# jhultman/vision3d

Measured on AMD Instinct MI355X. Metric: frames/sec SECOND fwd, 16k-pt KITTI cloud, higher is better.
Workload: dtype f16x3-scaled (fp32-class): fp32 operands split into f16 hi + lo pieces of x * s under per-tensor power-of-two scales, 3 MFMA terms (lo*hi + hi*lo + hi*hi), fp32 accumulate; relative product error 2^-22 -- the result differs from the reference's fp32 modules by fp32 summation noise: strict elementwis

## Files before the change

vision3d_amd/csrc/spconv.hip:

```cpp
#include "v3d_internal.h"

#include "sp_device.h"
#include "rb_device.h"

#define SP_RIDER_PROLOGUE(lds)                                                                        \
  if (rider.blocks && (int)blockIdx.x < rider.blocks) {                                               \
    if (threadIdx.x < V3D_BLOCK) rb_rider_run(rider, (int)blockIdx.x, (unsigned char*)(lds));         \
    return;                                                                                           \
  }                                                                                                   \
  const int bid = (int)blockIdx.x - rider.blocks;                                                     \
  [[maybe_unused]] const int nblk = (int)gridDim.x - rider.blocks;



__global__ __launch_bounds__(V3D_BLOCK) void spconv_fwd_scalar(const float* __restrict__ in,
                                                               const float* __restrict__ W,
                                                               const int* __restrict__ nbr,
                                                               const int* __restrict__ n_ptr, int cap, int K, int Cin,
                                                               int Cout, const float* __restrict__ scale,
                                                               const float* __restrict__ shift, int relu,
                                                               float* __restrict__ out) {
  const int n = min(*n_ptr, cap);
  const long long total = (long long)n * Cout;
  for (long long t = (long long)blockIdx.x * V3D_BLOCK + threadIdx.x; t < total; t += (long long)gridDim.x * V3D_BLOCK) {
// ... 931 lines not shown

template <int CIN, int COUT, int OG, int NBUF, int NMV, int ALOOK, int STAGE, int TILES, int PREC, int INS>
__device__ __forceinline__ void spconv_ring_body(const float* __restrict__ in, const unsigned short* __restrict__ wimg,
                                                 const int* __restrict__ nbr, const int n, int cap, const float* __restrict__ scale,
                                                 const float* __restrict__ shift, int relu, float* __restrict__ out, const int wg_in,
                                                 const SpScales& ss, float& vmax, unsigned short* __restrict__ out_s, const float s_next,
                                                 unsigned char* __restrict__ wb0 ) {
  constexpr int K = 27, ROUNDS = (K + OG - 1) / OG, NCW = TILES * OG;
  constexpr int LOOK = NBUF - 1;
  constexpr int ABUF = ALOOK + 1;
  constexpr int KI = CIN / 32, NB = COUT / 16;
  constexpr int NF = KI * NB * 2;
  constexpr int WBYTES = NF * 1024;
  constexpr int RB = OG * WBYTES;
  constexpr int FPM = OG * NF / NMV;
  constexpr int NSTG = (ROUNDS + 3) / 4;
  static_assert(CIN % 32 == 0 && CIN <= 128 && (OG * NF) % NMV == 0 && (LOOK - 1) * FPM < 64, "shape not covered by the ring kernel");
  static_assert(RB >= TILES * OG * NB * 4 * 64 * 4, "partials must fit one round buffer");
  static_assert(ALOOK >= 1 && ALOOK <= 4 && (ALOOK * KI * 2 <= 8 || ALOOK * KI * 2 == 12 || ALOOK * KI * 2 == 16), "gather look-ahead");
  __shared__ __attribute__((aligned(16))) unsigned char wb1[RB];
  __shared__ __attribute__((aligned(16))) unsigned char wb2[NBUF >= 3 ? RB : 16];
  __shared__ __attribute__((aligned(16))) unsigned char wb3[NBUF == 4 ? RB : 16];
  __shared__ int nbr_all[TILES * K * 16];
  __shared__ __attribute__((aligned(16))) unsigned char aslot[STAGE ? NCW * ALOOK * CIN * 64 : 16];
#define SPR_RING(i) ((i) % NBUF == 0 ? wb0 : ((i) % NBUF == 1 ? wb1 : ((i) % NBUF == 2 ? wb2 : wb3)))
  const int tid = threadIdx.x, lane = tid & 63;
  const int wv = __builtin_amdgcn_readfirstlane(tid >> 6);
  int wg = wg_in;
  {
    const int nwg = (n + 16 * TILES - 1) / (16 * TILES);
    const int qd = nwg / 8, rmd = nwg % 8, xcd = wg % 8, idx = wg / 8;
    wg = (xcd < rmd ? xcd * (qd + 1) : rmd * (qd + 1) + (xcd - rmd) * qd) + idx;
  }

  [[maybe_unused]] const int wave = wv == NCW ? 3 : (wv < 3 ? wv : 99);
  SPR_STAMP(0);
  if (wv >= NCW) {
    typedef const __attribute__((address_space(1))) void* gptr_t;
    typedef __attribute__((address_space(3))) void* lptr_t;
    const int mv = wv - NCW;
    const unsigned char* wsrc = reinterpret_cast<const unsigned char*>(wimg) + (size_t)mv * FPM * 1024 + (size_t)lane * 16;
#define SPR_DMA(R)                                                                                                  \
  {                                                                                                                 \
    const unsigned char* gsrc = wsrc + (size_t)(R) * RB;                                                            \
    _Pragma("unroll") for (int i = 0; i < FPM; i++) {                                                               \
      const bool ok = (R) * OG + (mv * FPM + i) / NF < K;                                                           \
      __builtin_amdgcn_global_load_lds((gptr_t)(gsrc + i * 1024 - (ok ? 0 : WBYTES)),                               \
                                       (lptr_t)(SPR_RING(R) + (mv * FPM + i) * 1024), 16, 0, 0);                    \
    }                                                                                                               \
  }
#pragma unroll
    for (int R = 0; R < LOOK; R++) SPR_DMA(R)
    SPR_STAMP(1);
#pragma unroll
    for (int R = 0; R < ROUNDS; R++) {
      const int younger = (ROUNDS - 1 - R) < (LOOK - 1) ? (ROUNDS - 1 - R) : (LOOK - 1);
      if (younger == 2) asm volatile("s_waitcnt vmcnt(%0)\n\ts_barrier" ::"n"(2 * FPM < 64 ? 2 * FPM : 63) : "memory");
      else if (younger == 1) asm volatile("s_waitcnt vmcnt(%0)\n\ts_barrier" ::"n"(FPM) : "memory");
      else asm volatile("s_waitcnt vmcnt(0)\n\ts_barrier" ::: "memory");
      if (R + LOOK < ROUNDS) SPR_DMA(R + LOOK)
      SPR_STAMP(3 + (R < 9 ? R : 8));
    }
#undef SPR_DMA
    __syncthreads();
    return;
  }

  const int t = wv / OG, g = wv % OG;
  int* nbr_s = nbr_all + t * K * 16;
  const int row0 = (wg * TILES + t) * 16;
  const int r = lane & 15, kg = lane >> 4;
  f32x4 araw[STAGE ? 1 : ABUF][KI * 2];
  f32x4 acc[NB];
#pragma unroll
  for (int j = 0; j < NB; j++) acc[j] = f32x4{0.f, 0.f, 0.f, 0.f};
  const int rsel = STAGE ? (lane >> 2) : r;
  const float* prow = spr_zero_row;
  auto row_ptr = [&](int src_i) {
    const int src = src_i;
    prow = (src >= 0 ? in + (size_t)src * CIN : spr_zero_row) + (STAGE ? ((lane & 3) ^ ((lane >> 5) & 1)) * 4 : (INS ? kg * 4 : kg * 8));
  };
  const unsigned slot0 = STAGE ? __builtin_amdgcn_readfirstlane(lds_addr_of(aslot) + wv * (ALOOK * CIN * 64)) : 0u;
  auto issue_chunk = [&](int ki, int Rr) {
    if constexpr (STAGE) {
      asm_dma16(prow + (ki * 2) * 16, slot0 + (Rr % ALOOK) * (CIN * 64) + (ki * 2) * 1024);
      asm_dma16(prow + (ki * 2 + 1) * 16, slot0 + (Rr % ALOOK) * (CIN * 64) + (ki * 2 + 1) * 1024);
    } else {
      f32x4 (&a)[KI * 2] = araw[Rr % ABUF];
      if constexpr (INS) {
        if (ki == 0) {
          asm_gld16(a[0], prow);
          if constexpr (CIN == 64) asm_gld16_128(a[1], prow);
          else asm_gld16_64(a[1], prow);
        } else if constexpr (KI == 2) {
          asm_gld16_64(a[2], prow);
          asm_gld16_192(a[3], prow);
        }
      } else if (ki == 0) {
        asm_gld16(a[0], prow);
        asm_gld16_16(a[1], prow);
      } else if constexpr (KI == 2) {
        asm_gld16_128(a[2], prow);
        asm_gld16_144(a[3], prow);
      }
    }
  };
  int nsrc = -1;
  {
    const bool live = row0 + r < n;
    int first[ALOOK], stage[NSTG];
#pragma unroll
    for (int i = 0; i < ALOOK; i++) first[i] = (row0 + rsel < n && i * OG + g < K) ? nbr[(size_t)(i * OG + g) * cap + row0 + rsel] : -1;
#pragma unroll
    for (int i = 0; i < NSTG; i++) {
      const int kk = (kg + 4 * i) * OG + g;
      stage[i] = (live && kk < K) ? nbr[(size_t)kk * cap + row0 + r] : -1;
    }
#pragma unroll
    for (int i = 0; i < ALOOK; i++) {
      row_ptr(first[i]);
#pragma unroll
      for (int ki = 0; ki < KI; ki++) issue_chunk(ki, i);
    }
#pragma unroll
    for (int i = 0; i < NSTG; i++)
      if ((kg + 4 * i) * OG + g < K) nbr_s[((kg + 4 * i) * OG + g) * 16 + r] = stage[i];
    if (ALOOK < ROUNDS && ALOOK * OG + g < K) nsrc = nbr_s[(ALOOK * OG + g) * 16 + rsel];
  }
  SPR_STAMP(1);
#pragma unroll
  for (int R = 0; R < ROUNDS; R++) {
    asm volatile("s_waitcnt lgkmcnt(0)\n\ts_barrier" ::: "memory");
    if (R + ALOOK < ROUNDS) row_ptr(nsrc);
    if (R + ALOOK + 1 < ROUNDS) nsrc = ((R + ALOOK + 1) * OG + g < K) ? nbr_s[((R + ALOOK + 1) * OG + g) * 16 + rsel] : -1;
    {
      const int younger = (ROUNDS - 1 - R < ALOOK - 1 ? ROUNDS - 1 - R : ALOOK - 1) * KI * 2;
      if constexpr (STAGE) {
        if (younger == 0) vm_wait<0>();
        else if (younger == 2) vm_wait<2>();
        else if (younger == 4) vm_wait<4>();
        else if (younger == 6) vm_wait<6>();
        else if (younger == 8) vm_wait<8>();
        else vm_wait<12>();
        const int sw = (r >> 3) & 1;
        const unsigned char* sl = aslot + (wv * ALOOK + R % ALOOK) * (CIN * 64) + (INS ? r * 64 + ((kg ^ sw) * 16) : (kg >> 1) * 1024 + r * 64);
#pragma unroll
        for (int ki = 0; ki < KI; ki++)
#pragma unroll
          for (int v = 0; v < 2; v++)
            araw[0][ki * 2 + v] = INS ? *reinterpret_cast<const f32x4*>(sl + (v * KI + ki) * 1024)
                                      : *reinterpret_cast<const f32x4*>(sl + ki * 2048 + ((((kg & 1) * 2 + v) ^ sw) * 16));
      } else {
        f32x4 (&ar)[KI * 2] = araw[R % ABUF];
        if (younger == 0) vm_wait_tie<0>(ar);
        else if (younger == 2) vm_wait_tie<2>(ar);
        else if (younger == 4) vm_wait_tie<4>(ar);
        else if (younger == 6) vm_wait_tie<6>(ar);
        else if (younger == 8) vm_wait_tie<8>(ar);
        else if (younger == 12) vm_wait_tie<12>(ar);
        else vm_wait_tie<16>(ar);
      }
    }
    const u32x4_t* bw = reinterpret_cast<const u32x4_t*>(SPR_RING(R) + g * WBYTES) + lane;
    u32x4_t ah[KI], al[KI], bh[KI][NB], bl[KI][NB];
#pragma unroll
    for (int ki = 0; ki < KI; ki++)
#pragma unroll
      for (int j = 0; j < NB; j++) {
        bh[ki][j] = bw[(size_t)((ki * NB + j) * 2) * 64];
        bl[ki][j] = bw[(size_t)((ki * NB + j) * 2 + 1) * 64];
      }
#pragma unroll
    for (int ki = 0; ki < KI; ki++) {
      const f32x4 v0 = araw[STAGE ? 0 : R % ABUF][ki * 2], v1 = araw[STAGE ? 0 : R % ABUF][ki * 2 + 1];
      const float x[8] = {v0.x, v0.y, v0.z, v0.w, v1.x, v1.y, v1.z, v1.w};
      split_in<PREC, INS>(x, ss.s_in, ah[ki], al[ki]);
    }
#pragma unroll
    for (int ki = 0; ki < KI; ki++) {
#pragma unroll
      for (int j = 0; j < NB; j++) acc[j] = sp_mfma<PREC>(al[ki], bh[ki][j], acc[j]);
#pragma unroll
      for (int j = 0; j < NB; j++) acc[j] = sp_mfma<PREC>(ah[ki], bl[ki][j], acc[j]);
#pragma unroll
      for (int j = 0; j < NB; j++) acc[j] = sp_mfma<PREC>(ah[ki], bh[ki][j], acc[j]);
      if (R + ALOOK < ROUNDS) {
        __builtin_amdgcn_sched_barrier(0);
        issue_chunk(ki, R + ALOOK);
        __builtin_amdgcn_sched_barrier(0);
      }
    }
#if SPR_TIMELINE
    __builtin_amdgcn_sched_barrier(0);
    SPR_STAMP(3 + (R < 9 ? R : 8));
#endif
  }
  float* part = reinterpret_cast<float*>((ROUNDS - 1) % NBUF != 0 ? wb0 : wb1) + t * (OG * NB * 4 * 64);
#pragma unroll
  for (int j = 0; j < NB; j++)
#pragma unroll
    for (int rr = 0; rr < 4; rr++) part[((g * NB + j) * 4 + rr) * 64 + lane] = acc[j][rr];
  SPR_STAMP(12);
  __syncthreads();
  SPR_STAMP(13);
  for (int it = g; it < NB * 4; it += OG) {
    const int j = it >> 2, rr = it & 3;
    const int col = j * 16 + r, row = row0 + kg * 4 + rr;
    float v = part[((0 * NB + j) * 4 + rr) * 64 + lane];
#pragma unroll
    for (int w = 1; w < OG; w++) v += part[((w * NB + j) * 4 + rr) * 64 + lane];
    if (row < n) {
      if (scale) v = v * (scale[col] * ss.undo) + shift[col];
      else if constexpr (PREC == 1) v = v * ss.undo;
      if (relu) v = fmaxf(v, 0.f);
      if constexpr (PREC == 1) vmax = fmaxf(vmax, fabsf(v));
      if (out) out[(size_t)row * COUT + col] = v;
      if (out_s) sp_store_split<PREC, COUT>(out_s, row, col, r, v, s_next);
    }
  }
  SPR_STAMP(14);
#undef SPR_RING
}

template <int CIN, int COUT, int OG, int NBUF, int NMV, int ALOOK, int STAGE, int TILES, int PREC, int INS>
__global__ __launch_bounds__((TILES * OG + NMV) * 64) void spconv_fwd_rows_ring(const float* __restrict__ in,
                                                                          const unsigned short* __restrict__ wimg,
                                                                          const int* __restrict__ nbr,
                                                                          const int* __restrict__ n_ptr, int cap,
                                                                          const float* __restrict__ scale,
                                                                          const float* __restrict__ shift, int relu,
                                                                          float* __restrict__ out, const V3dActScale as,
                                                                          unsigned short* __restrict__ out_s, const RbScanJob rider) {
  constexpr int RB0 = OG * (CIN / 32) * (COUT / 16) * 2 * 1024;
  static_assert(RB0 >= RB_SCAN_LDS, "a rider's scratch fits round buffer 0");
  __shared__ __attribute__((aligned(16))) unsigned char wb0[RB0];
  constexpr bool HOST = !(CIN == 64 && COUT == 64);
  int bid = (int)blockIdx.x, nblk = (int)gridDim.x;
  if constexpr (HOST) {
    if (rider.blocks && bid < rider.blocks) {
      if (threadIdx.x < V3D_BLOCK) rb_rider_run(rider, bid, wb0);
      return;
    }
    bid -= rider.blocks;
    nblk -= rider.blocks;
  }
  const int n = min(*n_ptr, cap);
  const int nwg = (n + 16 * TILES - 1) / (16 * TILES);
  const SpScales ss = sp_scales<PREC>(as, wimg, (size_t)27 * (CIN / 32) * (COUT / 16) * 2 * 512);
  const float s_next = (PREC == 1 && out_s) ? as.next[0] : 1.f;
  float vmax = 0.f;
  for (int g = bid; g < nwg; g += nblk) {
    spconv_ring_body<CIN, COUT, OG, NBUF, NMV, ALOOK, STAGE, TILES, PREC, INS>(in, wimg, nbr, n, cap, scale, shift, relu, out, g, ss, vmax,
                                                                              out_s, s_next, wb0);
    __syncthreads();
  }
  if constexpr (PREC == 1) sp_range_check(as, vmax, ss.limit);
}

struct SpLaunch {
  int prec;
  V3dActScale as;
  const void* in_split;
  unsigned short* out_split;
  const RbScanJob* rider;
  bool* rider_taken;
};

static RbScanJob sp_ring_rider(const SpLaunch& sl, int max_blocks) {
  if (!sl.rider || max_blocks < 1 || sl.rider->blocks > max_blocks) return RbScanJob{};
  return *sl.rider;
}

template <int CIN, int COUT, int OG, int NBUF, int NMV, int ALOOK, int STAGE, int TILES, int PREC, int INS>
static int launch_rows_ring_p(const float* in, const void* wimg, const int* nbr, const int* n_ptr, int cap,
                              const float* scale, const float* shift, int relu, float* out, hipStream_t st, const SpLaunch& sl) {
  static V3dPerDeviceInt cache;
  int* slots = cache.slot();
  if (!*slots) {
    int dev = 0, n_cu = 0, per_cu = 0;
    V3D_CHECK_HIP(hipGetDevice(&dev));
    V3D_CHECK_HIP(hipDeviceGetAttribute(&n_cu, hipDeviceAttributeMultiprocessorCount, dev));
    V3D_CHECK_HIP(hipOccupancyMaxActiveBlocksPerMultiprocessor(&per_cu, spconv_fwd_rows_ring<CIN, COUT, OG, NBUF, NMV, ALOOK, STAGE, TILES, PREC, INS>,
                                                               (TILES * OG + NMV) * 64, 0));
    *slots = std::max(8, per_cu * n_cu / 8 * 8);
  }
  const RbScanJob r = sp_ring_rider(sl, CIN == 64 && COUT == 64 ? 0 : 512);
  const int grid = std::min(v3d_ceil_div(cap, 16 * TILES), std::max(*slots - r.blocks, 8));
  hipLaunchKernelGGL((spconv_fwd_rows_ring<CIN, COUT, OG, NBUF, NMV, ALOOK, STAGE, TILES, PREC, INS>), dim3(grid + r.blocks),
                     dim3((TILES * OG + NMV) * 64), 0, st, INS ? (const float*)sl.in_split : in, (const unsigned short*)wimg, nbr, n_ptr, cap,
                     scale, shift, relu, out, sl.as, sl.out_split, r);
  if (sl.rider_taken) *sl.rider_taken = r.blocks > 0;
  V3D_CHECK_LAUNCH();
  return V3D_OK;
}
template <int CIN, int COUT, int OG, int NBUF, int NMV, int ALOOK = 2, int STAGE = 0, int TILES = 2>
static int launch_rows_ring(const float* in, const void* wimg, const int* nbr, const int* n_ptr, int cap,
                            const float* scale, const float* shift, int relu, float* out, hipStream_t st, const SpLaunch& sl) {
#define V3D_RING(P, I) launch_rows_ring_p<CIN, COUT, OG, NBUF, NMV, ALOOK, STAGE, TILES, P, I>(in, wimg, nbr, n_ptr, cap, scale, shift, relu, out, st, sl)
  if (sl.prec == V3D_PREC_F16S) return sl.in_split ? V3D_RING(1, 1) : V3D_RING(1, 0);
  return sl.in_split ? V3D_RING(0, 1) : V3D_RING(0, 0);
#undef V3D_RING
}

template <int CIN, int COUT, int PREC, int INS>
static void launch_rows_big(const float* in, const void* wimg, const int* nbr, const int* n_ptr, int cap, int K,
                            const float* scale, const float* shift, int relu, float* out, hipStream_t st, const SpLaunch& sl) {
  constexpr int NF = ((CIN + 31) / 32) * (COUT / 16) * 2;
  const size_t lds = std::max((size_t)2 * NF * 64 * 16 + (size_t)K * 64 * 4, (size_t)4 * SP_STAGE_BYTES(COUT));
  hipLaunchKernelGGL((spconv_fwd_rows_big<CIN, COUT, PREC, INS>), dim3(v3d_ceil_div(cap, 64)), dim3(V3D_BLOCK), lds, st,
                     INS ? (const float*)sl.in_split : in, (const unsigned short*)wimg, nbr, n_ptr, cap, K, scale, shift, relu, out, sl.as,
                     sl.out_split);
}

template <int CIN, int COUT, int T, int STAGE, int PREC, int INS>
static void launch_rows_kouter(const float* in, const void* wimg, const int* nbr, const int* n_ptr, int cap,
                               const float* scale, const float* shift, int relu, float* out, hipStream_t st, const SpLaunch& sl) {
  const int passes = v3d_ceil_div(cap, 16 * (T == 3 ? 2 : T) * 8);
  const int grid = passes >= 256 ? 256 : ((passes + 7) / 8) * 8;
  hipLaunchKernelGGL((spconv_fwd_rows_kouter<CIN, COUT, T, 27, STAGE, PREC, INS>), dim3(grid), dim3(512), 0, st,
                     INS ? (const float*)sl.in_split : in, (const unsigned short*)wimg, nbr, n_ptr, cap, scale, shift, relu, out, sl.as,
                     sl.out_split);
}

#define V3D_BIG_ROWS 32768
#define V3D_RING_ROWS 16384
template <int CIN, int COUT, int PREC, int INS>
static int launch_rows(const float* in, const void* wimg, const int* nbr, const int* n_ptr, int cap, int K,
                       const float* scale, const float* shift, int relu, float* out, int rows_hint, hipStream_t st,
                       const V3dDensifyOut* densify, int tiles_min, const SpLaunch& sl) {
  const int force = densify ? 1 : (rows_hint < 0 ? -rows_hint : 0);
  if constexpr (CIN >= 32 && CIN <= 64 && COUT >= 32 && COUT <= 64) {
    if (K == 27 && (force == 6 || force == 7 || force == 8 || (force == 0 && CIN == 64 && COUT == 64 && rows_hint >= V3D_BIG_ROWS))) {
      if (force == 7) launch_rows_kouter<CIN, COUT, 2, 0, PREC, INS>(in, wimg, nbr, n_ptr, cap, scale, shift, relu, out, st, sl);
      else if (force == 8) launch_rows_kouter<CIN, COUT, 2, 1, PREC, INS>(in, wimg, nbr, n_ptr, cap, scale, shift, relu, out, st, sl);
      else launch_rows_kouter<CIN, COUT, 3, 1, PREC, INS>(in, wimg, nbr, n_ptr, cap, scale, shift, relu, out, st, sl);
      V3D_CHECK_LAUNCH();
      return V3D_OK;
    }
    if (force == 5 || (force == 0 && rows_hint >= V3D_BIG_ROWS)) {
      launch_rows_big<CIN, COUT, PREC, INS>(in, wimg, nbr, n_ptr, cap, K, scale, shift, relu, out, st, sl);
      V3D_CHECK_LAUNCH();
      return V3D_OK;
    }
    if (K == 27 && (force == 10 || force == 16 || (force >= 12 && force <= 14) || (force == 0 && rows_hint <= V3D_RING_ROWS))) {
      if constexpr (CIN == 64 && COUT == 64) {
        if (force != 16) {
          const long long want = force ? 0 : (long long)rows_hint + rows_hint / 10;
          int tiles = force == 12 ? 2 : force == 13 ? 3 : force == 14 ? 4 : (want <= 32 * 256 ? 2 : want <= 48 * 256 ? 3 : 4);
          if (!force && tiles < tiles_min) tiles = tiles_min > 4 ? 4 : tiles_min;
          if (tiles == 2) return launch_rows_ring<CIN, COUT, 3, 2, 4, 1, 1, 2>(in, wimg, nbr, n_ptr, cap, scale, shift, relu, out, st, sl);
          if (tiles == 3) return launch_rows_ring<CIN, COUT, 3, 2, 4, 1, 1, 3>(in, wimg, nbr, n_ptr, cap, scale, shift, relu, out, st, sl);
          return launch_rows_ring<CIN, COUT, 3, 2, 4, 1, 1, 4>(in, wimg, nbr, n_ptr, cap, scale, shift, relu, out, st, sl);
        }
      }
      if (force != 16 && CIN == 32 && COUT == 32) return launch_rows_ring<CIN, COUT, 3, 2, 2, 2, 1>(in, wimg, nbr, n_ptr, cap, scale, shift, relu, out, st, sl);
      return launch_rows_ring<CIN, COUT, 3, 3, 2>(in, wimg, nbr, n_ptr, cap, scale, shift, relu, out, st, sl);
    }
  }
  const size_t lds = std::max((size_t)4 * (COUT / 16) * 4 * 64 * 4 + (size_t)K * 16 * 4 + 2 * SP_STAGE_BYTES(COUT),
                              (size_t)RB_SCAN_LDS);
  const RbScanJob r = sl.rider ? *sl.rider : RbScanJob{};
  hipLaunchKernelGGL((spconv_fwd_rows<CIN, COUT, PREC, INS>), dim3(v3d_ceil_div(cap, 16) + r.blocks), dim3(V3D_BLOCK), lds, st,
                     INS ? (const float*)sl.in_split : in, (const unsigned short*)wimg, nbr, n_ptr, cap, K, scale, shift, relu, out,
                     densify ? *densify : V3dDensifyOut{}, sl.as, sl.out_split, r);
  if (sl.rider_taken) *sl.rider_taken = r.blocks > 0;
  V3D_CHECK_LAUNCH();
  return V3D_OK;
}

extern "C" int v3d_sparse_conv_fwd_packed(const float* in, const void* weight_image, const int32_t* nbr,
                                           const int32_t* n_out, int cap_out, int K, int Cin, int Cout, const float* scale,
                                           const float* shift, int relu, float* out, int rows_hint, int prec,
                                           const float* act_in, const float* act_next, int32_t* range_flag,
                                           const void* in_split, void* out_split, v3d_stream_t stream) {
  const V3dActScale as{act_in, act_next, range_flag, nullptr};
  return v3d_i_sparse_conv_fwd_packed(in ? in : (const float*)in_split, weight_image, nbr, n_out, cap_out, K, Cin, Cout, scale, shift,
                                      relu, out, rows_hint, (hipStream_t)stream, nullptr, 2, prec, &as, in_split, out_split);
}

template <int PREC>
__global__ __launch_bounds__(256) void rows_split_kernel(const float* __restrict__ rows, const int* __restrict__ n_ptr, int cap, int C,
                                                         const float* __restrict__ entry, unsigned short* __restrict__ out) {
  const long long total = (long long)(n_ptr ? min(*n_ptr, cap) : cap) * C;
  const float s = PREC == 1 ? entry[0] : 1.f;
  for (long long t = (long long)blockIdx.x * 256 + threadIdx.x; t < total; t += (long long)gridDim.x * 256) {
    const long long row = t / C;
    const int c = (int)(t - row * C);
    unsigned short h, l;
    split_one<PREC>(rows[t], s, h, l);
    out[row * 2 * C + c] = h;
    out[row * 2 * C + C + c] = l;
  }
}

extern "C" int v3d_sparse_rows_split(const float* rows, const int32_t* n_rows, int cap, int C, int prec, const float* act_entry,
                                     void* out_split, v3d_stream_t stream) {
  if (!rows || !out_split || cap < 1 || C < 8 || C % 8) return V3D_EINVAL;
  if (prec == V3D_PREC_F16S ? !act_entry : prec != V3D_PREC_BF16X3) return V3D_EINVAL;
  const int blocks = (int)std::min<long long>(((long long)cap * C + 255) / 256, 4096);
  if (prec == V3D_PREC_F16S)
    hipLaunchKernelGGL(rows_split_kernel<1>, dim3(blocks), dim3(256), 0, (hipStream_t)stream, rows, n_rows, cap, C, act_entry, (unsigned short*)out_split);
  else
    hipLaunchKernelGGL(rows_split_kernel<0>, dim3(blocks), dim3(256), 0, (hipStream_t)stream, rows, n_rows, cap, C, nullptr, (unsigned short*)out_split);
  V3D_CHECK_LAUNCH();
  return V3D_OK;
}

bool v3d_i_sparse_conv_packed_supported(int Cin, int Cout) {
  static const int shapes[][2] = {{4, 16}, {16, 16}, {16, 32}, {32, 32}, {32, 64}, {64, 64}, {4, 32}, {32, 16}, {64, 32}, {64, 128}, {128, 128}};
  for (const auto& s : shapes)
    if (s[0] == Cin && s[1] == Cout) return true;
  return false;
}

int v3d_i_sparse_conv_fwd_packed(const float* in, const void* weight_image, const int32_t* nbr, const int32_t* n_out,
                                 int cap_out, int K, int Cin, int Cout, const float* scale, const float* shift, int relu,
                                 float* out, int rows_hint, hipStream_t st, const V3dDensifyOut* densify, int ring_tiles_min,
                                 int prec, const V3dActScale* act, const void* in_split, void* out_split, const RbScanJob* rider,
                                 bool* rider_taken) {
  if (rider_taken) *rider_taken = false;
  if (!in || !weight_image || !nbr || !n_out || (!out && !out_split) || cap_out < 1 || K < 1) return V3D_EINVAL;
  if ((scale == nullptr) != (shift == nullptr)) return V3D_EINVAL;
  if (!out && densify) return V3D_EINVAL;
  if (prec != V3D_PREC_BF16X3 && prec != V3D_PREC_F16S) return V3D_EINVAL;
  if (prec == V3D_PREC_F16S && (!act || !act->in || ((densify || out_split) && !act->next))) return V3D_EINVAL;
  if (in_split && Cin % 8) return V3D_EINVAL;
  SpLaunch sl;
  sl.prec = prec;
  sl.as = (prec == V3D_PREC_F16S) ? *act : V3dActScale{nullptr, nullptr, nullptr, nullptr};
  sl.in_split = in_split;
  sl.out_split = (unsigned short*)out_split;
  sl.rider = rider;
  sl.rider_taken = rider_taken;
#define V3D_GO(ci, co, P, I) \
  return launch_rows<ci, co, P, I>(in, weight_image, nbr, n_out, cap_out, K, scale, shift, relu, out, rows_hint, st, densify, ring_tiles_min, sl)
#define V3D_TRY(ci, co)                                    \
  if (Cin == ci && Cout == co) {                           \
    if constexpr ((ci) % 8 == 0) {                         \
      if (prec == V3D_PREC_F16S && in_split) V3D_GO(ci, co, 1, 1); \
      if (prec == V3D_PREC_BF16X3 && in_split) V3D_GO(ci, co, 0, 1); \
    }                                                      \
    if (prec == V3D_PREC_F16S) V3D_GO(ci, co, 1, 0);       \
    V3D_GO(ci, co, 0, 0);                                  \
  }
  V3D_TRY(4, 16)
  V3D_TRY(16, 16)
  V3D_TRY(16, 32)
  V3D_TRY(32, 32)
  V3D_TRY(32, 64)
  V3D_TRY(64, 64)
  V3D_TRY(4, 32)
  V3D_TRY(32, 16)
  V3D_TRY(64, 32)
  V3D_TRY(64, 128)
  V3D_TRY(128, 128)
#undef V3D_TRY
#undef V3D_GO
  return V3D_EUNSUPPORTED;
}

extern "C" int v3d_sparse_conv_fwd(const float* in, const float* weight, const int32_t* nbr, const int32_t* n_out,
                                   int cap_out, int K, int Cin, int Cout, const float* scale, const float* shift,
                                   int relu, float* out, int algo, v3d_stream_t stream) {
  return v3d_i_sparse_conv_fwd_exact(in, weight, nbr, n_out, cap_out, K, Cin, Cout, scale, shift, relu, out, algo, (hipStream_t)stream,
                                     nullptr, nullptr, nullptr, nullptr, nullptr);
}

int v3d_i_sparse_conv_fwd_exact(const float* in, const float* weight, const int32_t* nbr, const int32_t* n_out, int cap_out, int K,
                                int Cin, int Cout, const float* scale, const float* shift, int relu, float* out, int algo,
                                hipStream_t st, const float* next_entry, int32_t* range_flag, unsigned* seen, const RbScanJob* rider,
                                bool* rider_taken) {
  if (rider_taken) *rider_taken = false;
  if (!in || !weight || !nbr || !n_out || !out || cap_out < 1 || K < 1 || Cin < 1 || Cout < 1) return V3D_EINVAL;
  if ((scale == nullptr) != (shift == nullptr)) return V3D_EINVAL;
  if (algo != 0 && algo != 1 && algo != 3) return V3D_EINVAL;
  if (algo == 0 || algo == 3) {
    int rc = V3D_EUNSUPPORTED;
#define V3D_TRY(ci, co) \
  if (Cin == ci && Cout == co) rc = launch_wave<ci, co>(in, weight, nbr, n_out, cap_out, K, scale, shift, relu, out, st, next_entry, range_flag, seen, rider, rider_taken);
    V3D_TRY(4, 16)
    V3D_TRY(16, 16)
    V3D_TRY(16, 32)
    V3D_TRY(32, 32)
    V3D_TRY(32, 64)
    V3D_TRY(64, 64)
    V3D_TRY(4, 32)
    V3D_TRY(32, 16)
    V3D_TRY(64, 32)
    V3D_TRY(64, 128)
    V3D_TRY(128, 128)
#undef V3D_TRY
    if (rc != V3D_EUNSUPPORTED || algo == 3) return rc;
  }
  const long long total = (long long)cap_out * Cout;
  const int blocks = (int)((total + V3D_BLOCK - 1) / V3D_BLOCK);
  hipLaunchKernelGGL(spconv_fwd_scalar, dim3(blocks > 8192 ? 8192 : blocks), dim3(V3D_BLOCK), 0, st, in, weight, nbr,
                       n_out, cap_out, K, Cin, Cout, scale, shift, relu, out);
  V3D_CHECK_LAUNCH();
  return V3D_OK;
}

#define BW_MAX_SPLITS 64
#define BW_Q 128

__host__ __device__ static inline int bw_rows_per_block(int n) {
  const int r = ((n + BW_MAX_SPLITS - 1) / BW_MAX_SPLITS + 255) & ~255;
  return r < 256 ? 256 : r;
}

template <int TI, int TJ>
__global__ __launch_bounds__(V3D_BLOCK) void spconv_bwd_weight_tiles(const float* __restrict__ X,
                                                                     const float* __restrict__ dY,
                                                                     const int* __restrict__ nbr,
                                                                     const int* __restrict__ n_ptr, int cap, int Cin,
                                                                     int Cout, int groups_j,
                                                                     float* __restrict__ partial ) {
  __shared__ int q_src[4][BW_Q];
  __shared__ int q_out[4][BW_Q];
  __shared__ float red[TI * TJ * 256];
  const int n = min(*n_ptr, cap);
  const int rows_per_block = bw_rows_per_block(n);
  const int slab = blockIdx.x, k = blockIdx.y, K = gridDim.y;
  const int lo = slab * rows_per_block;
  if (lo >= n) return;
  const int hi = min(n, lo + rows_per_block);
  const int ci_base = (blockIdx.z / groups_j) * TI * 16, co_base = (blockIdx.z % groups_j) * TJ * 16;
  const int lane = threadIdx.x & 63, wave = threadIdx.x >> 6;
  const int r = lane & 15, p = lane >> 4;
  const int rows_per_wave = rows_per_block >> 2;
  const int wlo = lo + wave * rows_per_wave, whi = min(hi, wlo + rows_per_wave);
  const int* __restrict__ nk = nbr + (size_t)k * cap;
  int* qs = q_src[wave];
  int* qo = q_out[wave];

  f32x4 acc[TI][TJ];
#pragma unroll
  for (int t = 0; t < TI; t++)
#pragma unroll
    for (int u = 0; u < TJ; u++) acc[t][u] = f32x4{0.f, 0.f, 0.f, 0.f};

  auto consume = [&](int base, int valid) {
    float a[4][TI], b[4][TJ];
#pragma unroll
    for (int s4 = 0; s4 < 4; s4++) {
      const int e = 4 * s4 + p;
      const bool ok = e < valid;
      const int src = ok ? qs[base + e] : 0, o = ok ? qo[base + e] : 0;
#pragma unroll
      for (int t = 0; t < TI; t++) {
        const int ci = ci_base + 16 * t + r;
        a[s4][t] = (ok && ci < Cin) ? X[(size_t)src * Cin + ci] : 0.f;
      }
#pragma unroll
      for (int u = 0; u < TJ; u++) {
        const int co = co_base + 16 * u + r;
        b[s4][u] = (ok && co < Cout) ? dY[(size_t)o * Cout + co] : 0.f;
      }
    }
#pragma unroll
    for (int s4 = 0; s4 < 4; s4++)
#pragma unroll
      for (int t = 0; t < TI; t++)
#pragma unroll
        for (int u = 0; u < TJ; u++) acc[t][u] = __builtin_amdgcn_mfma_f32_16x16x4f32(a[s4][t], b[s4][u], acc[t][u], 0, 0, 0);
  };

  int cnt = 0;
  int src_next = (wlo < whi && wlo + lane < whi) ? nk[wlo + lane] : -1;
  for (int o0 = wlo; o0 < whi; o0 += 64) {
    const int src = src_next;
    const int o = o0 + lane;
    src_next = (o + 64 < whi) ? nk[o + 64] : -1;
    const unsigned long long live = __ballot(src >= 0);
    if (src >= 0) {
      const int pos = cnt + __popcll(live & ((1ull << lane) - 1ull));
      qs[pos] = src;
      qo[pos] = o;
    }
    cnt += __popcll(live);
    int g = 0;
    for (; cnt - g >= 16; g += 16) consume(g, 16);
    if (g) {
      const int rem = cnt - g;
      int ms = 0, mo = 0;
      if (lane < rem) { ms = qs[g + lane]; mo = qo[g + lane]; }
      if (lane < rem) { qs[lane] = ms; qo[lane] = mo; }
      cnt = rem;
    }
  }
  if (cnt > 0) consume(0, cnt);

  for (int w = 0; w < 4; w++) {
    if (wave == w) {
#pragma unroll
      for (int t = 0; t < TI; t++)
#pragma unroll
        for (int u = 0; u < TJ; u++)
#pragma unroll
          for (int rr = 0; rr < 4; rr++) {
            const int idx = (((t * TJ + u) * 4 + rr) << 6) + lane;
            red[idx] = w == 0 ? acc[t][u][rr] : red[idx] + acc[t][u][rr];
          }
    }
    __syncthreads();
  }
  float* outp = partial + ((size_t)slab * K + k) * Cin * Cout;
  for (int idx = threadIdx.x; idx < TI * TJ * 256; idx += V3D_BLOCK) {
    const int l = idx & 63, rr = (idx >> 6) & 3, tu = idx >> 8;
    const int ci = ci_base + 16 * (tu / TJ) + (l >> 4) * 4 + rr;
    const int co = co_base + 16 * (tu % TJ) + (l & 15);
    if (ci < Cin && co < Cout) outp[(size_t)ci * Cout + co] = red[idx];
  }
}

__global__ void spconv_bwd_weight_reduce_kernel(const float* __restrict__ partial, const int* __restrict__ n_ptr, int cap,
                                                long long elems, float* __restrict__ dW) {
  const int n = min(*n_ptr, cap);
  const int rows_per_block = bw_rows_per_block(n);
  const int slabs = (n + rows_per_block - 1) / rows_per_block;
  for (long long i = (long long)blockIdx.x * blockDim.x + threadIdx.x; i < elems; i += (long long)gridDim.x * blockDim.x) {
    float s = 0.f;
    for (int sp = 0; sp < slabs; sp++) s += partial[(size_t)sp * elems + i];
    dW[i] = s;
  }
}

extern "C" size_t v3d_sparse_conv_bwd_weight_workspace(int K, int Cin, int Cout) {
  return (size_t)BW_MAX_SPLITS * K * Cin * Cout * sizeof(float) + 256;
}

template <int TI, int TJ>
static void launch_bwd_weight(const float* X, const float* dY, const int* nbr, const int* n_out, int cap, int K, int Cin,
                              int Cout, int slabs, float* partial, hipStream_t st) {
  const int gi = ((Cin + 15) / 16 + TI - 1) / TI, gj = ((Cout + 15) / 16 + TJ - 1) / TJ;
  hipLaunchKernelGGL((spconv_bwd_weight_tiles<TI, TJ>), dim3(slabs, K, gi * gj), dim3(V3D_BLOCK), 0, st, X, dY, nbr, n_out,
                     cap, Cin, Cout, gj, partial);
}

extern "C" int v3d_sparse_conv_bwd_weight(const float* X, const float* dY, const int32_t* nbr, const int32_t* n_out,
                                          int cap_out, int K, int Cin, int Cout, float* dW, void* workspace,
                                          size_t workspace_bytes, v3d_stream_t stream) {
  hipStream_t st = (hipStream_t)stream;
  if (!X || !dY || !nbr || !n_out || !dW || !workspace || cap_out < 1 || K < 1 || K > 65535 || Cin < 1 || Cout < 1)
    return V3D_EINVAL;
  if (workspace_bytes < v3d_sparse_conv_bwd_weight_workspace(K, Cin, Cout)) return V3D_EWORKSPACE;
  const int slabs = std::min(BW_MAX_SPLITS, v3d_ceil_div(cap_out, 256));
  const int ti = Cin > 32 ? 4 : (Cin > 16 ? 2 : 1), tj = Cout > 32 ? 4 : (Cout > 16 ? 2 : 1);
  float* partial = (float*)workspace;
// ... 40 lines not shown
```

Measured before the change: 4762.

## Add LDS-resident-weight sparse conv kernel for 64x64 small-row layers

Adds a new sparse-conv kernel for 64->64 channel, K=27 layers. Each block DMAs the weight slice for one 16-column output group of all 27 offsets into LDS once, then loops persistently over row chunks assigned per XCD, prefetching gathered input rows two offsets ahead and rotating three accumulators. It becomes the default path for 64x64 layers below the ring-row threshold, replacing the ring kernel and its rider scan-job co-scheduling. The intent is to avoid reloading weights per tile and to improve locality, at the cost of large LDS use and lower occupancy.

```diff
diff --git a/vision3d_amd/csrc/spconv.hip b/vision3d_amd/csrc/spconv.hip
--- a/vision3d_amd/csrc/spconv.hip
+++ b/vision3d_amd/csrc/spconv.hip
@@ -1257,6 +1257,181 @@
 #undef V3D_RING
 }
 
+typedef int spres_rsrc_t __attribute__((ext_vector_type(4)));
+#define SPRES_ABSENT 0x80000000u
+template <int OFF> __device__ __forceinline__ void asm_bld16(f32x4& d, const unsigned voff, const spres_rsrc_t rsrc) {
+  asm volatile("buffer_load_dwordx4 %0, %1, %2, 0 offen offset:%3" : "=v"(d) : "v"(voff), "s"(rsrc), "n"(OFF) : "memory");
+}
+#define SPRES_WAVES 16
+template <int PREC, int INS>
+__global__ __launch_bounds__(SPRES_WAVES * 64) void spconv_fwd_rows_resident(const float* __restrict__ in,
+                                                                            const unsigned short* __restrict__ wimg,
+                                                                            const int* __restrict__ nbr, const int* __restrict__ n_ptr,
+                                                                            int cap, const float* __restrict__ scale,
+                                                                            const float* __restrict__ shift, int relu,
+                                                                            float* __restrict__ out, const V3dActScale as,
+                                                                            unsigned short* __restrict__ out_s) {
+  constexpr int CIN = 64, COUT = 64, K = 27, KI = CIN / 32, NB = COUT / 16;
+  constexpr int NF = KI * 2;
+  constexpr int PF = 2;
+  __shared__ __attribute__((aligned(16))) unsigned char wsl[K * NF * 1024];
+  __shared__ int idx_s[SPRES_WAVES][K * 16];
+  const int tid = threadIdx.x, lane = tid & 63;
+  const int wv = __builtin_amdgcn_readfirstlane(tid >> 6);
+  const int bid = (int)blockIdx.x, nblk = (int)gridDim.x;
+  const int n = min(*n_ptr, cap);
+  const int per_round = nblk / NB;
+  int T = ((n + 15) / 16 + per_round - 1) / per_round;
+  T = min(SPRES_WAVES, max(4, (T + 3) & ~3));
+  const int nck = (n + 16 * T - 1) / (16 * T);
+  const int xcd = bid & 7, j = (bid >> 3) & 3;
+  const int qd = nck / 8, rmd = nck % 8;
+  const int run0 = xcd < rmd ? xcd * (qd + 1) : rmd * (qd + 1) + (xcd - rmd) * qd, run_n = qd + (xcd < rmd ? 1 : 0);
+  if ((bid >> 5) >= run_n) return;
+
+  const SpScales ss = sp_scales<PREC>(as, wimg, (size_t)K * KI * NB * 2 * 512);
+  const float s_next = (PREC == 1 && out_s) ? as.next[0] : 1.f;
+  {
+    const unsigned char* wsrc = reinterpret_cast<const unsigned char*>(wimg) + j * 2048 + lane * 16;
+    const unsigned wdst = lds_addr_of(wsl);
+    for (int f = wv; f < K * NF; f += SPRES_WAVES) {
+      const int k = f / NF, ki = (f / 2) % KI, piece = f % 2;
+      asm_dma16(wsrc + (size_t)k * (KI * NB * 2 * 1024) + ki * (NB * 2 * 1024) + piece * 1024, __builtin_amdgcn_readfirstlane(wdst + f * 1024));
+    }
+    asm volatile("s_waitcnt vmcnt(0)\n\ts_barrier" ::: "memory");
+  }
+  float vmax = 0.f;
+  const int r = lane & 15, kg = lane >> 4;
+  int* my_idx = idx_s[wv];
+  const u32x4_t* bw = reinterpret_cast<const u32x4_t*>(wsl) + lane;
+  for (int local = bid >> 5; local < run_n; local += nblk >> 5) {
+    const int row0 = (run0 + local) * 16 * T + wv * 16;
+    if (wv >= T || row0 >= n) break;
+    {
+      const bool live = row0 + r < n;
+      int v[(K + 3) / 4];
+#pragma unroll
+      for (int i = 0; i < (K + 3) / 4; i++) {
+        const int k = kg + 4 * i;
+        v[i] = (live && k < K) ? nbr[(size_t)k * cap + row0 + r] : -1;
+      }
+#pragma unroll
+      for (int i = 0; i < (K + 3) / 4; i++)
+        if (kg + 4 * i < K) my_idx[(kg + 4 * i) * 16 + r] = v[i];
+    }
+    f32x4 araw[PF + 1][KI * 2];
+    auto issue = [&](int k, int src) {
+      const float* prow = (src >= 0 ? in + (size_t)src * CIN : spr_zero_row) + (INS ? kg * 4 : kg * 8);
+      f32x4 (&a)[KI * 2] = araw[k % (PF + 1)];
+      if constexpr (INS) {
+        asm_gld16(a[0], prow);
+        asm_gld16_128(a[1], prow);
+        asm_gld16_64(a[2], prow);
+        asm_gld16_192(a[3], prow);
+      } else {
+        asm_gld16(a[0], prow);
+        asm_gld16_16(a[1], prow);
+        asm_gld16_128(a[2], prow);
+        asm_gld16_144(a[3], prow);
+      }
+    };
+    auto read_b = [&](int k, u32x4_t (&b)[KI][2]) {
+#pragma unroll
+      for (int ki = 0; ki < KI; ki++)
+#pragma unroll
+        for (int p = 0; p < 2; p++) b[ki][p] = bw[((k * KI + ki) * 2 + p) * 64];
+    };
+    f32x4 acc[3];
+#pragma unroll
+    for (int g = 0; g < 3; g++) acc[g] = f32x4{0.f, 0.f, 0.f, 0.f};
+#pragma unroll
+    for (int k = 0; k < PF; k++) issue(k, my_idx[k * 16 + r]);
+    int src_next = my_idx[PF * 16 + r];
+    u32x4_t bcur[KI][2], bnext[KI][2];
+    read_b(0, bcur);
+#pragma unroll
+    for (int k = 0; k < K; k++) {
+      if (k + PF < K) {
+        issue(k + PF, src_next);
+        if (k + PF + 1 < K) src_next = my_idx[(k + PF + 1) * 16 + r];
+      }
+      f32x4 (&a)[KI * 2] = araw[k % (PF + 1)];
+      {
+        const int younger = (K - 1 - k < PF ? K - 1 - k : PF) * KI * 2;
+        if (younger == 0) vm_wait_tie<0>(a);
+        else if (younger == 4) vm_wait_tie<4>(a);
+        else vm_wait_tie<8>(a);
+      }
+      if (k + 1 < K) read_b(k + 1, bnext);
+      u32x4_t ah[KI], al[KI];
+#pragma unroll
+      for (int ki = 0; ki < KI; ki++) {
+        const float x[8] = {a[ki * 2].x, a[ki * 2].y, a[ki * 2].z, a[ki * 2].w, a[ki * 2 + 1].x, a[ki * 2 + 1].y, a[ki * 2 + 1].z, a[ki * 2 + 1].w};
+        split_in<PREC, INS>(x, ss.s_in, ah[ki], al[ki]);
+      }
+      f32x4& d = acc[k % 3];
+#pragma unroll
+      for (int ki = 0; ki < KI; ki++) {
+        d = sp_mfma<PREC>(al[ki], bcur[ki][0], d);
+        d = sp_mfma<PREC>(ah[ki], bcur[ki][1], d);
+        d = sp_mfma<PREC>(ah[ki], bcur[ki][0], d);
+      }
+      if (k + 1 < K) {
+#pragma unroll
+        for (int ki = 0; ki < KI; ki++) {
+          bcur[ki][0] = bnext[ki][0];
+          bcur[ki][1] = bnext[ki][1];
+        }
+      }
+    }
+    const int col = j * 16 + r;
+    const float sc = scale ? scale[col] * ss.undo : 1.f, sh = scale ? shift[col] : 0.f;
+#pragma unroll
+    for (int rr = 0; rr < 4; rr++) {
+      const int row = row0 + kg * 4 + rr;
+      float v = acc[0][rr] + acc[1][rr];
+      v += acc[2][rr];
+      if (row < n) {
+        if (scale) v = v * sc + sh;
+        else if constexpr (PREC == 1) v = v * ss.undo;
+        if (relu) v = fmaxf(v, 0.f);
+        if constexpr (PREC == 1) vmax = fmaxf(vmax, fabsf(v));
+        if (out) out[(size_t)row * COUT + col] = v;
+        if (out_s) sp_store_split<PREC, COUT>(out_s, row, col, r, v, s_next);
+      }
+    }
+  }
+  if constexpr (PREC == 1) sp_range_check(as, vmax, ss.limit);
+}
+
+template <int PREC, int INS>
+static int launch_rows_resident_p(const float* in, const void* wimg, const int* nbr, const int* n_ptr, int cap, const float* scale,
+                                  const float* shift, int relu, float* out, hipStream_t st, const SpLaunch& sl) {
+  static V3dPerDeviceInt cache;
+  int* slots = cache.slot();
+  if (!*slots) {
+    int dev = 0, n_cu = 0, per_cu = 0;
+    V3D_CHECK_HIP(hipGetDevice(&dev));
+    V3D_CHECK_HIP(hipDeviceGetAttribute(&n_cu, hipDeviceAttributeMultiprocessorCount, dev));
+    V3D_CHECK_HIP(hipOccupancyMaxActiveBlocksPerMultiprocessor(&per_cu, spconv_fwd_rows_resident<PREC, INS>, SPRES_WAVES * 64, 0));
+    *slots = std::max(32, per_cu * n_cu / 32 * 32);
+  }
+  const int grid = std::min(v3d_ceil_div(v3d_ceil_div(cap, 64), 8) * 32, *slots);
+  hipLaunchKernelGGL((spconv_fwd_rows_resident<PREC, INS>), dim3(grid), dim3(SPRES_WAVES * 64), 0, st,
+                     INS ? (const float*)sl.in_split : in, (const unsigned short*)wimg, nbr, n_ptr, cap, scale, shift, relu, out, sl.as,
+                     sl.out_split);
+  V3D_CHECK_LAUNCH();
+  return V3D_OK;
+}
+static int launch_rows_resident(const float* in, const void* wimg, const int* nbr, const int* n_ptr, int cap, const float* scale,
+                                const float* shift, int relu, float* out, hipStream_t st, const SpLaunch& sl) {
+  if (sl.prec == V3D_PREC_F16S)
+    return sl.in_split ? launch_rows_resident_p<1, 1>(in, wimg, nbr, n_ptr, cap, scale, shift, relu, out, st, sl)
+                       : launch_rows_resident_p<1, 0>(in, wimg, nbr, n_ptr, cap, scale, shift, relu, out, st, sl);
+  return sl.in_split ? launch_rows_resident_p<0, 1>(in, wimg, nbr, n_ptr, cap, scale, shift, relu, out, st, sl)
+                     : launch_rows_resident_p<0, 0>(in, wimg, nbr, n_ptr, cap, scale, shift, relu, out, st, sl);
+}
+
 template <int CIN, int COUT, int PREC, int INS>
 static void launch_rows_big(const float* in, const void* wimg, const int* nbr, const int* n_ptr, int cap, int K,
                             const float* scale, const float* shift, int relu, float* out, hipStream_t st, const SpLaunch& sl) {
@@ -1297,8 +1472,9 @@
       V3D_CHECK_LAUNCH();
       return V3D_OK;
     }
-    if (K == 27 && (force == 10 || force == 16 || (force >= 12 && force <= 14) || (force == 0 && rows_hint <= V3D_RING_ROWS))) {
+    if (K == 27 && (force == 10 || force == 16 || (force >= 12 && force <= 14) || force == 18 || (force == 0 && rows_hint <= V3D_RING_ROWS))) {
       if constexpr (CIN == 64 && COUT == 64) {
+        if (force == 18 || force == 0) return launch_rows_resident(in, wimg, nbr, n_ptr, cap, scale, shift, relu, out, st, sl);
         if (force != 16) {
           const long long want = force ? 0 : (long long)rows_hint + rows_hint / 10;
           int tiles = force == 12 ? 2 : force == 13 ? 3 : force == 14 ? 4 : (want <= 32 * 256 ? 2 : want <= 48 * 256 ? 3 : 4);
```

New measurement: 3562, median of 2. 25.2% lower.
